# CSRavasio/oflibpytorch

Hardware: AMD Instinct MI355X
Metric: Mpix/s warped+composed (Flow(...) x2 from raw tensors, Flow.apply 't' C=3 + valid area, then Flow.combine_with mode=3 -- the methods combine_flows / apply_flow wrap -- 1080p fp32) (higher is better)
Workload: dtype f32; 1 GPU; B=64/GPU 1080x1920 fp32: Flow(f,'t',mask) x2 (validation), Flow.apply('t', C=3 image, target+flow masks, valid area) + combine_with(mode=3, 't', masks); batch_per_gpu=64, global_batch=64, height=1080, width=1920, parallelism=batch-sharded x1 (no data-path collective), launcher=single process, bytes_per_px=62

## Files before the change

### include/oflib_hip.h

```cpp
#ifndef OFLIB_HIP_H
#define OFLIB_HIP_H

#include <stdint.h>

#ifdef __cplusplus
extern "C" {
#endif

#define OFL_OK 0
#define OFL_E_NULL -1
#define OFL_E_SHAPE -2
#define OFL_E_ARG -3
#define OFL_E_UNSUPPORTED -4

int ofl_version(void);

#define OFL_OPT_WARP_PATH 1
#define OFL_OPT_WARP_SHEAR 3
#define OFL_OPT_SPLAT_PASS_IMAGES 4
#define OFL_OPT_SPLAT_FALLBACK_SLOTS 5
#define OFL_OPT_SPLAT_EXTRA_LDS 7
int ofl_set_option(int32_t key, int32_t value);
const char* ofl_last_kernel_name(void);

// ... 76 lines not shown
                            const uint8_t* chan_mask_a, int64_t chan_mask_a_bs,
                            const uint8_t* chan_mask_b, int64_t chan_mask_b_bs,
                            int32_t with_mask_chan, int32_t occlude,
                            float* dst, float* density, uint8_t* warped, uint8_t* valid, float* mask_chan,
                            int32_t* workspace, int64_t workspace_ints, float* accum_fallback,
                            int32_t n, int32_t c, int32_t h, int32_t w,
                            int32_t round_mode, void* stream);

int ofl_splat_sum_f32(const float* flow, int64_t flow_bs, float flow_sign,
                      const float* data, int64_t data_bs, float data_sign, float* dst,
                      int32_t* workspace, int64_t workspace_ints, float* accum_fallback,
                      int32_t n, int32_t c, int32_t h, int32_t w, void* stream);

#define OFL_FLAG_NONFINITE 1
#define OFL_FLAG_NZ 2
#define OFL_FLAG_NZ_THR 4
#define OFL_FLAG_NZ_MASKED 8
#define OFL_FLAG_NZ_THR_MASKED 16

int ofl_flow_flags_f32(const float* flow, int64_t flow_bs,
                       const uint8_t* mask, int64_t mask_bs, float thr,
                       int32_t* flags, int32_t n, int32_t h, int32_t w, void* stream);

#define OFL_FLAGS_HOST_WORK_EXTRA 33
int ofl_flow_flags_host(const void* flow, int32_t flow_is_f16, int64_t flow_bs,
                        const uint8_t* mask, int64_t mask_bs, float thr,
                        int32_t* work, int32_t* host_words, int32_t serial,
                        int32_t n, int32_t h, int32_t w, void* stream);
int ofl_host_words_alloc(int64_t ints, void** out);
int ofl_host_words_free(void* ptr);

int ofl_flow_from_f16(const void* src_f16, int64_t src_bs,
                      const uint8_t* mask, int64_t mask_bs,
                      float* dst, int32_t* flags,
                      int32_t n, int32_t h, int32_t w, void* stream);
int ofl_splat_tiled_f16(const void* flow_f16, int64_t flow_bs, float flow_sign,
                        const void* data_f16, int64_t data_bs, float data_sign,
                        const uint8_t* weight_mask, int64_t weight_mask_bs,
                        const uint8_t* chan_mask_a, int64_t chan_mask_a_bs,
                        const uint8_t* chan_mask_b, int64_t chan_mask_b_bs,
                        int32_t with_mask_chan, int32_t occlude,
                        void* dst, int32_t dst_is_f16, uint8_t* valid, int32_t* dst_flags,
                        int32_t* workspace, int64_t workspace_ints, float* accum_fallback,
                        int32_t n, int32_t h, int32_t w, void* stream);
int ofl_warp_bwd_h_f32(const float* flow, int64_t flow_bs, float flow_sign,
                       const void* src_f16, int64_t src_bs,
                       const float* src_b, int64_t src_b_bs,
                       const uint8_t* src_mask, int64_t src_mask_bs,
                       const uint8_t* flow_mask, int64_t flow_mask_bs,
                       float* dst, uint8_t* valid,
                       int32_t n, int32_t h, int32_t w, void* stream);

#define OFL_X16_HALF 0
// ... 136 lines not shown
```

### oflibpytorch_amd/_build.py

```python
import os
import shutil
import subprocess

_PKG = os.path.dirname(os.path.abspath(__file__))
_ROOT = os.path.dirname(_PKG)
SOURCES = [os.path.join(_PKG, "csrc", "ofl_kernels.hip"), os.path.join(_PKG, "csrc", "ofl_aux_kernels.hip"), os.path.join(_PKG, "csrc", "ofl_splat_gather.hip"),
           os.path.join(_PKG, "csrc", "ofl_warp_wide.hip"), os.path.join(_PKG, "csrc", "ofl_visualise.hip"), os.path.join(_PKG, "csrc", "ofl_matrix.hip"),
           os.path.join(_PKG, "csrc", "ofl_arrows.hip"), os.path.join(_PKG, "csrc", "ofl_mesh.hip"), os.path.join(_PKG, "csrc", "ofl_warp_half.hip"),
           os.path.join(_PKG, "csrc", "ofl_warp_nhwc.hip"), os.path.join(_PKG, "csrc", "ofl_loaders.hip"), os.path.join(_PKG, "csrc", "ofl_metrics.hip"),
           os.path.join(_PKG, "csrc", "ofl_consistency.hip"),
           os.path.join(_PKG, "csrc", "ofl_png_host.cpp")]
HEADERS = [os.path.join(_ROOT, "include", "oflib_hip.h")]
LIB_PATH = os.path.join(_PKG, "libofl_hip.so")

HIPCC_FLAGS = ["-O3", "--offload-arch=gfx950", "-std=c++17", "-fPIC", "-shared", "-ffp-contract=off",
               "-fno-fast-math", "-fvisibility=hidden"]


def hipcc_path() -> str:
    for cand in (os.environ.get("HIPCC"), shutil.which("hipcc"), "/opt/rocm/bin/hipcc"):
        if cand and os.path.exists(cand):
            return cand
    raise RuntimeError("oflibpytorch_amd: hipcc not found (set HIPCC or install ROCm under /opt/rocm)")


def needs_build() -> bool:
    if not os.path.exists(LIB_PATH):
        return True
    t = os.path.getmtime(LIB_PATH)
    return any(os.path.getmtime(s) > t for s in SOURCES + HEADERS)


def build(force: bool = False, verbose: bool = False) -> str:
    if not force and not needs_build():
# ... 39 lines not shown
```

### oflibpytorch_amd/_native.py

```python
import ctypes
import math
import os
import threading
import time

import numpy as np
import torch

from . import _build

FLAG_NONFINITE, FLAG_NZ, FLAG_NZ_THR, FLAG_NZ_MASKED, FLAG_NZ_THR_MASKED = 1, 2, 4, 8, 16
ABI_VERSION = 36
ROUND_NONE, ROUND_RINT, ROUND_U8 = 0, 1, 2
THRESHOLD = 1e-3

_SYMBOLS = ("ofl_version", "ofl_set_option", "ofl_warp_bwd_f32", "ofl_splat_fwd_f32", "ofl_splat_finalize_f32", "ofl_splat_tiled_workspace_ints", "ofl_splat_tiled_pass_images",
            "ofl_splat_tiled_f32", "ofl_flow_flags_f32", "ofl_warp_bwd_u8", "ofl_flow_from_f16",
            "ofl_warp_bwd_grad_f32", "ofl_splat_grad_f32", "ofl_sample_pts_f32", "ofl_sample_pts_grad_f32",
            "ofl_flow_extents_f32", "ofl_flag_words_or_i32", "ofl_splat_sum_f32", "ofl_warp_bwd_win_f32", "ofl_splat_tiled_win_f32", "ofl_splat_tiled_f16",
            "ofl_warp_bwd_h_f32", "ofl_flow_flags_host", "ofl_host_words_alloc", "ofl_host_words_free", "ofl_flow_from_matrix_f32", "ofl_splat_tiled_fallback_images", "ofl_warp_valid_f32", "ofl_resize_bilinear_f32", "ofl_splat_tile_geometry", "ofl_splat_gather_info", "ofl_last_kernel_name",
            "ofl_visualise_workspace_ints", "ofl_visualise_range_f32", "ofl_visualise_u8",
            "ofl_matrix_workspace_bytes", "ofl_matrix_fit_f64",
            "ofl_arrows_workspace_ints", "ofl_arrows_scale_f32", "ofl_arrows_plan", "ofl_arrows_u8",
            "ofl_mesh_workspace_ints", "ofl_mesh_plan", "ofl_mesh_apply", "ofl_mesh_points",
            "ofl_warp_bwd_x16", "ofl_warp_bwd_grad_x16", "ofl_splat_sum_x16", "ofl_warp_bwd_nhwc",
            "ofl_warp_bwd_grad_nhwc", "ofl_nhwc_to_planes", "ofl_planes_to_nhwc",
            "ofl_png_unfilter", "ofl_png_grey8", "ofl_decode_kitti", "ofl_decode_flo",
            "ofl_flow_error_workspace_bytes", "ofl_flow_error_f64", "ofl_flow_epe_grad_f32",
            "ofl_flow_consistency_workspace_bytes", "ofl_flow_consistency_f32")
_lib = None
_load_lock = threading.RLock()


class NativeUnavailable(RuntimeError):
    """The HIP backend (libofl_hip.so + a visible HIP device) is required and missing."""


def load_library(path: str = None):
    if _lib is not None and path is None:
        return _lib
    with _load_lock:
        return _load_library_locked(path)

# ... 41 lines not shown
    lib.ofl_splat_tiled_pass_images.argtypes = [i32, i32, i32]
    lib.ofl_splat_tiled_fallback_images.argtypes = [i32, i32, i32, i32]
    lib.ofl_splat_tile_geometry.argtypes = [p, p, p]
    lib.ofl_splat_gather_info.argtypes = [i32, i32, i32, i32, i32, p]
    lib.ofl_splat_tiled_f32.argtypes = [p, i64, f32, p, p, i64, p, i64, f32, p, i64, p, i64, p, i64, p, i64, i32, i32, p, p, p, p, p,
                                        p, p, i64, p, i32, i32, i32, i32, i32, p]
    lib.ofl_warp_bwd_grad_f32.argtypes = [p, i64, f32, p, i64, p, f32, p, i64, p, i32, i32, i32, i32, p]
    lib.ofl_splat_grad_f32.argtypes = [p, i64, f32, p, p, i64, p, i64, p, i64, i32, p, p, p, p, p, p, p, i32, i32, i32, i32, p]
    lib.ofl_sample_pts_f32.argtypes = [p, i64, p, i64, p, i32, i32, i32, i32, p]
    lib.ofl_sample_pts_grad_f32.argtypes = [p, i64, p, i64, p, p, p, i32, i32, i32, i32, p]
    lib.ofl_flow_extents_f32.argtypes = [p, i64, p, i64, f32, p, p, i32, i32, i32, p]
    lib.ofl_warp_valid_f32.argtypes = [p, i64, f32, p, i64, f32, p, i32, i32, i32, p]
    lib.ofl_resize_bilinear_f32.argtypes = [p, p, i32, i32, i32, i32, i32, f32, f32, p]
    lib.ofl_flag_words_or_i32.argtypes = [p, i32, p, p]
    lib.ofl_splat_sum_f32.argtypes = [p, i64, f32, p, i64, f32, p, p, i64, p, i32, i32, i32, i32, p]
    lib.ofl_splat_tiled_f16.argtypes = [p, i64, f32, p, i64, f32, p, i64, p, i64, p, i64, i32, i32, p, i32, p, p, p, i64, p, i32, i32, i32, p]
    lib.ofl_warp_bwd_h_f32.argtypes = [p, i64, f32, p, i64, p, i64, p, i64, p, i64, p, p, i32, i32, i32, p]
    lib.ofl_warp_bwd_win_f32.argtypes = [p, i64, f32, i32, i32, i32, i32, p, i64, p, i64, p, i64, p, p, i32, i32, i32, i32, i32, p]
    lib.ofl_splat_tiled_win_f32.argtypes = [p, i64, f32, i32, i32, i32, i32, p, i64, f32, p, i64, p, i64, p, i64, i32, i32, p, p, p, p, p,
                                            p, i64, p, i32, i32, i32, i32, i32, p]
    lib.ofl_flow_flags_host.argtypes = [p, i32, i64, p, i64, f32, p, p, i32, i32, i32, i32, p]
    lib.ofl_host_words_alloc.argtypes = [i64, ctypes.POINTER(ctypes.c_void_p)]
    lib.ofl_host_words_free.argtypes = [p]
    lib.ofl_flow_from_matrix_f32.argtypes = [p, i64, f32, p, i32, i32, i32, p]
    lib.ofl_visualise_workspace_ints.argtypes = [i32]
    lib.ofl_visualise_range_f32.argtypes = [p, i64, i32, p, i64, p, p, p, i32, i32, i32, p]
    lib.ofl_visualise_u8.argtypes = [p, i64, i32, p, i64, i32, i32, p, i32, i32, p, i32, i32, i32, p]
    lib.ofl_matrix_workspace_bytes.argtypes = [i32, i32, i32, i32, i32]
    lib.ofl_matrix_fit_f64.argtypes = [p, i64, i32, i32, p, i64, i32, i32, i32, i32, i32, p, p, p, p]
    lib.ofl_arrows_workspace_ints.argtypes = [i32, i32, i32, i32]
    lib.ofl_arrows_scale_f32.argtypes = [p, i64, i32, i32, p, p, i32, i32, i32, p]
    lib.ofl_arrows_plan.argtypes = [p, i64, i32, i32, i32, p, i32, i32, f32, p, i32, i32, i32, p]
    lib.ofl_arrows_u8.argtypes = [p, i64, i32, p, i64, i32, i32, i32, p, p, i64, i32, p, i32, i32, i32, p]
    lib.ofl_mesh_workspace_ints.argtypes = [i32, i32, i32, i32]
    lib.ofl_mesh_plan.argtypes = [p, i64, f32, p, i64, i32, p, i32, i32, i32, p]
    lib.ofl_mesh_apply.argtypes = [p, i64, f32, p, i64, p, i64, i32, i32, p, p, i64, p, p, p, i32, i32, i32, i32, i32, p]
    lib.ofl_mesh_points.argtypes = [p, i64, f32, p, i64, p, i64, p, p, i64, p, p, i32, i32, i32, i32, p]
    lib.ofl_warp_bwd_x16.argtypes = [p, i64, f32, p, i64, p, i64, p, i64, p, i64, p, i64, f32, f32, p, p, p, p, p,
                                     i32, i32, i32, i32, i32, i32, p]
    lib.ofl_warp_bwd_grad_x16.argtypes = [p, i64, f32, p, i64, p, f32, p, i32, i32, i32, i32, i32, p]
    lib.ofl_splat_sum_x16.argtypes = [p, i64, f32, p, i64, f32, p, p, i64, p, i32, i32, i32, i32, i32, p]
    lib.ofl_warp_bwd_nhwc.argtypes = [p, i64, f32, p, i64, p, i64, p, i64, p, p, i32, i32, i32, i32, i32, p]
    lib.ofl_warp_bwd_grad_nhwc.argtypes = [p, i64, f32, p, i64, p, f32, p, i32, i32, i32, i32, i32, p]
    lib.ofl_nhwc_to_planes.argtypes = [p, p, i32, i32, i32, i32, i32, p]
    lib.ofl_planes_to_nhwc.argtypes = [p, p, i32, i32, i32, i32, i32, p]
    lib.ofl_png_unfilter.argtypes = [p, i64, i32, i32, i32, i32, p, i64]
# ... 119 lines not shown
    lib, dev = load_library(), device(vecs, mask)
    n, _, h, w = vecs.shape
    if vecs.dtype == torch.float16 and vecs.device.type == 'cuda':
        with _on(dev):
            v, vbs = _planes(vecs.detach(), dev, torch.float16, n, "flow")
            if vbs != 0 or n == 1:
                m, mbs = (None, 0) if mask is None else _planes(mask, dev, torch.bool, n, "mask")
                flags = torch.zeros(n, dtype=torch.int32, device=dev)
                rc = lib.ofl_flow_from_f16(_ptr(v), vbs, _ptr(m), mbs, None, _ptr(flags), n, h, w, _stream(dev))
                if rc != -4:
                    _check(rc, "ofl_flow_from_f16")
                    return flags
        vecs = vecs.float()
    with _on(dev):
        v, vbs = _planes(vecs.detach(), dev, torch.float32, n, "flow")
        m, mbs = (None, 0) if mask is None else _planes(mask, dev, torch.bool, n, "mask")
        flags = torch.zeros(n, dtype=torch.int32, device=dev)
        _check(lib.ofl_flow_flags_f32(_ptr(v), vbs, _ptr(m), mbs, THRESHOLD, _ptr(flags), n, h, w, _stream(dev)),
               "ofl_flow_flags_f32")
    return flags


_HOST_WORDS = 1 << 12
_WORK_EXTRA = 33
_MAX_SLOTS = 8
_host_slots = {}
_host_slots_lock = threading.Lock()
_SPIN_SLACK_SECONDS = 150e-6
_YIELD_SECONDS = 20e-3
HOST_POLL_SECONDS = 20.0


def _new_host_slot(lib, dev):
    addr = ctypes.c_void_p()
    with torch.cuda.device(dev):
        _check(lib.ofl_host_words_alloc(2 * _HOST_WORDS, ctypes.byref(addr)), "ofl_host_words_alloc")
        work = torch.zeros(_HOST_WORDS + _WORK_EXTRA, dtype=torch.int32, device=dev)
    view = np.ctypeslib.as_array((ctypes.c_int32 * (2 * _HOST_WORDS)).from_address(addr.value))
    return [threading.Lock(), work, addr, view, 0, False]


def _acquire_host_slot(lib, dev):
    while True:
        slots = _host_slots.get(dev.index)
        if slots is not None:
            for slot in tuple(slots):
                if slot[0].acquire(False):
                    if slot[5]:
                        slot[0].release()
                        continue
                    return slot
        with _host_slots_lock:
            slots = _host_slots.setdefault(dev.index, [])
            if len(slots) < _MAX_SLOTS:
                slot = _new_host_slot(lib, dev)
                slot[0].acquire()
                slots.append(slot)
                return slot
            busy = slots[0]
        busy[0].acquire()
        if not busy[5]:
            return busy
# ... 13 lines not shown
        return None
    n, _, h, w = vecs.shape
    if n > _HOST_WORDS:
        return None
    lib, dev = load_library(), vecs.device
    half = vecs.dtype == torch.float16
    switch = torch.cuda.current_device() != dev.index
    ctx = torch.cuda.device(dev) if switch else None
    if ctx is not None:
        ctx.__enter__()
    try:
        if vecs.is_contiguous() and (mask is None or (mask.dtype == torch.bool and mask.device == dev and mask.shape[0] == n
                                                      and mask.is_contiguous())):
            v, vbs, m, mbs = vecs, 2 * h * w, mask, h * w
        else:
            v, vbs = _planes(vecs.detach(), dev, vecs.dtype, n, "flow")
            if half and vbs == 0 and n != 1:
                return None
            m, mbs = (None, 0) if mask is None else _planes(mask, dev, torch.bool, n, "mask")
        slot = _acquire_host_slot(lib, dev)
        stream = torch._C._cuda_getCurrentRawStream(dev.index)
        try:
            serial = slot[4] = (slot[4] % 0x7ffffff0) + 1
            view = slot[3]
            rc = lib.ofl_flow_flags_host(v.data_ptr(), 1 if half else 0, vbs, 0 if m is None else m.data_ptr(), mbs, THRESHOLD,
                                         slot[1].data_ptr(), slot[2], serial, n, h, w, stream)
            if rc == -4:
                return None
            _check(rc, "ofl_flow_flags_host")
            try:
                tags = view[0:2 * n:2]
                t0 = time.perf_counter()
                spin_until = t0 + 2.0 * (n * h * w * (5 if half else 9)) / 4e12 + _SPIN_SLACK_SECONDS
                looks = 0
                while not (view[2 * n - 2] == serial and (n == 1 or bool((tags == serial).all()))):
                    looks += 1
                    if looks & 0x3f == 0:
                        now = time.perf_counter()
                        if now > spin_until:
                            time.sleep(0 if now - t0 < _YIELD_SECONDS else 5e-5)
                            if now - t0 > HOST_POLL_SECONDS:
                                torch.cuda.synchronize(dev)
                                if bool((tags == serial).all()):
                                    break
                                raise RuntimeError("oflibpytorch_amd: the flag reduction did not report back")
                return view[1:2 * n:2].tolist()
            except BaseException:
                try:
                    torch.cuda.synchronize(dev)
                finally:
                    _drop_host_slot(dev, slot)
                raise
        finally:
            slot[0].release()
    finally:
        if ctx is not None:
            ctx.__exit__(None, None, None)


def flow_from_half(vecs16: torch.Tensor, mask: torch.Tensor = None):
    lib, dev = load_library(), device(vecs16, mask)
    n, _, h, w = vecs16.shape
    if _wants_grad(vecs16):
        dst = vecs16.to(dev).float()
        return dst, flow_flags(dst, mask)
    with _on(dev):
        v, vbs = _planes(vecs16, dev, torch.float16, n, "flow")
        if vbs != 0 or n == 1:
            m, mbs = (None, 0) if mask is None else _planes(mask, dev, torch.bool, n, "mask")
# ... 1034 lines not shown
```

### oflibpytorch_amd/csrc/ofl_kernels.hip

```cpp
#include <hip/hip_runtime.h>
#include <stdint.h>
#include <type_traits>

#include "oflib_hip.h"

#pragma clang fp contract(off)

int ofl_wide_launch_column(const void* params, int nc, void* stream);
int ofl_wide_launch_rows(const void* params, int nc, int tiles, void* stream);
int ofl_wide_launch_rows_h(const void* params, void* stream);
int ofl_wide_launch_rows_grad(const void* params, int nc, int tiles, void* stream);
int ofl_wide_launch_rows_u8(const void* params, int nc, int dst_is_u8, void* stream);
int ofl_wide_launch_chan(const void* params, int rows, void* stream);
int ofl_warp_path_option(void);
int ofl_warp_shear_option(void);
int ofl_splat_launch_gather_diet(const void* params, int nc, int mch, int elem, unsigned grid, void* stream, int extra_lds);

extern const void* g_ofl_last_kernel;
#define OFL_KLAUNCH(K, ...) do { g_ofl_last_kernel = (const void*)(K); hipLaunchKernelGGL(K, __VA_ARGS__); } while (0)

namespace {

constexpr float kValidThr = 0.99999f;
constexpr float kZeroThr = 1e-3f;
// ... 3043 lines not shown
            a0 = b0; b0 = min(a0 + span, ub);
        }
    }
    if (NC == 2 && s.dst_flags) {
        dflags = wave_or_flags(dflags);
        block_flag_or(&s.dst_flags[n], dflags);
    }
    if (!REDO) break;
#if OFL_SP2_UNITTIME
    if (tid == 0) {
        const uint64_t t1 = wall_clock64();
        p.redo_list[2 * ri] = tile | ((uint32_t)((unit_t0 >> 3) & 0xffffu) << 16);
        p.redo_list[2 * ri + 1] = (uint32_t)ua | ((uint32_t)ub << 8) | ((uint32_t)min((t1 - unit_t0) >> 2, (uint64_t)0xffffu) << 16);
    }
#endif
    if (tid == 0) next_unit = (int)gridDim.x + atomicAdd(&p.redo_cnt[1], 1);
    __syncthreads();
    ri = __builtin_amdgcn_readfirstlane(next_unit);
    } while (ri < redo_n);
#undef s
#undef p
}

constexpr int kFlagShards = 32;
struct FlagsHost { int32_t* counters; unsigned long long* host; int32_t serial, total_blocks, n; };

__device__ __forceinline__ void flags_publish(int32_t* __restrict__ flags, const FlagsHost& fh) {
    __shared__ int last;
    asm volatile("s_waitcnt vmcnt(0)" ::: "memory");
    __syncthreads();
    if (threadIdx.x == 0) {
        const int id = (int)(blockIdx.y * gridDim.x + blockIdx.x), shard = id % kFlagShards;
        const int in_shard = (fh.total_blocks - shard + kFlagShards - 1) / kFlagShards;
        const int shards = fh.total_blocks < kFlagShards ? fh.total_blocks : kFlagShards;
        int l = 0;
        if (__hip_atomic_fetch_add(fh.counters + shard, 1, __ATOMIC_RELAXED, __HIP_MEMORY_SCOPE_AGENT) == in_shard - 1)
            l = __hip_atomic_fetch_add(fh.counters + kFlagShards, 1, __ATOMIC_RELAXED, __HIP_MEMORY_SCOPE_AGENT) == shards - 1;
        last = l;
    }
    __syncthreads();
    if (!last) return;
    if (threadIdx.x <= kFlagShards) {
        const int old = __hip_atomic_exchange(fh.counters + threadIdx.x, 0, __ATOMIC_RELAXED, __HIP_MEMORY_SCOPE_AGENT);
        asm volatile("" :: "v"(old));
    }
    asm volatile("s_waitcnt vmcnt(0)" ::: "memory");
    __syncthreads();
    for (int i = threadIdx.x; i < fh.n; i += blockDim.x) {
        const uint32_t v = (uint32_t)__hip_atomic_exchange(&flags[i], 0, __ATOMIC_RELAXED, __HIP_MEMORY_SCOPE_AGENT);
        __hip_atomic_store(&fh.host[i], ((unsigned long long)v << 32) | (uint32_t)fh.serial, __ATOMIC_RELAXED, __HIP_MEMORY_SCOPE_SYSTEM);
    }
}

template <bool VEC, bool NT = false, bool HOST = false>
__global__ __launch_bounds__(256) void flow_flags_kernel(const float* __restrict__ flow, int64_t flow_bs,
                                                         const uint8_t* __restrict__ mask, int64_t mask_bs,
                                                         int32_t* __restrict__ flags, int64_t hw, const FlagsHost fh) {
    const int n = blockIdx.y;
    const float* fu = flow + n * flow_bs;
    const uint8_t* mk = mask ? mask + n * mask_bs : nullptr;
    int f = 0;
    const int64_t stride = (int64_t)gridDim.x * blockDim.x;
    if (VEC) {
        const int64_t hw4 = hw >> 2;
        constexpr int R = 4;
        bool skip_mask = false;
        for (int64_t i0 = (int64_t)blockIdx.x * blockDim.x + threadIdx.x; i0 < hw4; i0 += R * stride) {
            f4 a[R], b[R]; uint32_t m4[R];
#pragma unroll
            for (int r = 0; r < R; ++r) {
                const int64_t i = i0 + r * stride;
                if (i < hw4) {
                    if (NT) { a[r] = ld4nt(fu + 4 * i); b[r] = ld4nt(fu + hw + 4 * i); }
                    else { a[r] = reinterpret_cast<const f4*>(fu)[i]; b[r] = reinterpret_cast<const f4*>(fu + hw)[i]; }
                    m4[r] = (mk && !skip_mask) ? reinterpret_cast<const uint32_t*>(mk)[i] : 0x01010101u;
                }
            }
#pragma unroll
            for (int r = 0; r < R; ++r) {
                if (i0 + r * stride < hw4) {
#pragma unroll
                    for (int k = 0; k < 4; ++k) f |= flag_bits(a[r][k], b[r][k], ((m4[r] >> (8 * k)) & 0xffu) != 0u);
                }
            }
            if (mk && !skip_mask) skip_mask = __any((f & OFL_FLAG_NZ_THR_MASKED) != 0) != 0;
        }
    } else {
        for (int64_t i = (int64_t)blockIdx.x * blockDim.x + threadIdx.x; i < hw; i += stride)
            f |= flag_bits(fu[i], fu[hw + i], mk ? (mk[i] != 0) : true);
    }
    f = wave_or_flags(f);
    block_flag_or(&flags[n], f);
    if (HOST) flags_publish(flags, fh);
}

typedef _Float16 h4 __attribute__((ext_vector_type(4)));
template <bool HOST = false>
__global__ __launch_bounds__(256) void flow_f16_kernel(const _Float16* __restrict__ src, int64_t src_bs,
                                                       const uint8_t* __restrict__ mask, int64_t mask_bs,
                                                       float* __restrict__ dst, int32_t* __restrict__ flags, int64_t hw, const FlagsHost fh) {
    const int n = blockIdx.y;
    const _Float16* su = src + n * src_bs;
    float* du = dst + (int64_t)n * 2 * hw;
    const uint8_t* mk = mask ? mask + n * mask_bs : nullptr;
    int f = 0;
    const int64_t stride = (int64_t)gridDim.x * blockDim.x, hw4 = hw >> 2;
    for (int64_t i0 = (int64_t)blockIdx.x * blockDim.x + threadIdx.x; i0 < hw4; i0 += 4 * stride) {
        h4 a[4], b[4]; uint32_t m4[4];
#pragma unroll
        for (int r = 0; r < 4; ++r) {
            const int64_t i = i0 + r * stride;
            if (i < hw4) {
                a[r] = reinterpret_cast<const h4*>(su)[i]; b[r] = reinterpret_cast<const h4*>(su + hw)[i];
                m4[r] = mk ? reinterpret_cast<const uint32_t*>(mk)[i] : 0x01010101u;
            }
        }
#pragma unroll
        for (int r = 0; r < 4; ++r) {
            const int64_t i = i0 + r * stride;
            if (i < hw4) {
                const f4 u = {(float)a[r][0], (float)a[r][1], (float)a[r][2], (float)a[r][3]};
                const f4 v = {(float)b[r][0], (float)b[r][1], (float)b[r][2], (float)b[r][3]};
                if (dst) { reinterpret_cast<f4*>(du)[i] = u; reinterpret_cast<f4*>(du + hw)[i] = v; }
#pragma unroll
                for (int k = 0; k < 4; ++k) f |= flag_bits(u[k], v[k], ((m4[r] >> (8 * k)) & 0xffu) != 0u);
            }
        }
    }
    f = wave_or_flags(f);
    block_flag_or(&flags[n], f);
    if (HOST) flags_publish(flags, fh);
}

inline int check_dims(int32_t n, int32_t c, int32_t h, int32_t w, bool splat = true) {
    if (n < 1 || c < 1 || h < 1 || w < 1) return OFL_E_SHAPE;
    if (splat && (int64_t)h * w >= (1ll << 24)) return OFL_E_SHAPE;
    if ((int64_t)h * w >= (1ll << 31)) return OFL_E_SHAPE;
    return OFL_OK;
}

inline void tile_grid(int32_t n, int32_t h, int32_t w, int32_t& tiles_x, int32_t& tiles_y, int64_t& total,
                      int64_t& per_xcd, unsigned& grid) {
    tiles_x = (w + kTileW - 1) / kTileW;
    tiles_y = (h + kTileH - 1) / kTileH;
    total = (int64_t)tiles_x * tiles_y * n;
    per_xcd = (total + kXcds - 1) / kXcds;
    grid = (unsigned)(per_xcd * kXcds);
}

inline void magic_u32(uint32_t d, uint32_t& m, uint32_t& s) {
    uint32_t l = 0;
    while ((1ull << l) < d) ++l;
    m = (uint32_t)(((1ull << 32) * ((1ull << l) - d)) / d + 1);
    s = ((l ? 1u : 0u) << 16) | (l ? l - 1 : 0);
// ... 473 lines not shown
    return (int)hipGetLastError();
}

template <int NC, typename TD>
int launch_warp_lds_u8(WarpParams& q, hipStream_t st) {
    const unsigned g = warp_geometry(q, kLdsTWQ * 4, 2 * kLdsTH);
    OFL_WITH_BOOL(q.valid != nullptr, V, OFL_KLAUNCH((warp_bwd_lds_kernel<NC, V, false, false, false, uint8_t, TD>), dim3(g), dim3(kLdsNT), kLdsBytes, st, q));
    return (int)hipGetLastError();
}

inline bool aligned_to(const void* ptr, size_t a) { return (reinterpret_cast<uintptr_t>(ptr) % a) == 0; }

#ifndef OFL_FLAGS_BLOCKS
#define OFL_FLAGS_BLOCKS 512
#endif
void launch_flow_flags(const float* flow, int64_t flow_bs, const uint8_t* mask, int64_t mask_bs, int32_t* flags, int32_t n,
                       int64_t hw, hipStream_t st, const FlagsHost* fhp = nullptr) {
    const bool vec = (hw % 4) == 0 && aligned_to(flow, 16) && (flow_bs % 4) == 0 && (!mask || (aligned_to(mask, 4) && (mask_bs % 4) == 0));
    FlagsHost fh = {};
    if (fhp) fh = *fhp;
    if (vec) {
        int64_t bx = (hw / 4 + 1023) / 1024;
        int64_t cap = (n <= 8 ? OFL_FLAGS_BLOCKS / 2 : OFL_FLAGS_BLOCKS) / n;
        cap = cap < 16 ? 16 : (cap > 256 ? 256 : cap);
        if (bx > cap) bx = cap;
        fh.total_blocks = (int32_t)(bx * n);
        const bool nt = 9 * hw * n >= ((int64_t)256 << 20);
        if (fhp) {
            if (nt) OFL_KLAUNCH((flow_flags_kernel<true, true, true>), dim3((unsigned)bx, (unsigned)n), dim3(256), 0, st, flow, flow_bs, mask, mask_bs, flags, hw, fh);
            else OFL_KLAUNCH((flow_flags_kernel<true, false, true>), dim3((unsigned)bx, (unsigned)n), dim3(256), 0, st, flow, flow_bs, mask, mask_bs, flags, hw, fh);
        } else {
            if (nt) OFL_KLAUNCH((flow_flags_kernel<true, true>), dim3((unsigned)bx, (unsigned)n), dim3(256), 0, st, flow, flow_bs, mask, mask_bs, flags, hw, fh);
            else OFL_KLAUNCH((flow_flags_kernel<true, false>), dim3((unsigned)bx, (unsigned)n), dim3(256), 0, st, flow, flow_bs, mask, mask_bs, flags, hw, fh);
        }
    } else {
        int64_t bx = (hw + 255) / 256;
        if (bx > 512) bx = 512;
        fh.total_blocks = (int32_t)(bx * n);
        if (fhp) OFL_KLAUNCH((flow_flags_kernel<false, false, true>), dim3((unsigned)bx, (unsigned)n), dim3(256), 0, st, flow, flow_bs, mask, mask_bs, flags, hw, fh);
        else OFL_KLAUNCH((flow_flags_kernel<false>), dim3((unsigned)bx, (unsigned)n), dim3(256), 0, st, flow, flow_bs, mask, mask_bs, flags, hw, fh);
    }
}

template <int CT>
int launch_warp(const WarpParams& p, unsigned grid, hipStream_t st) {
    const bool valid = p.valid != nullptr, add = p.addend != nullptr, flags = p.flow_flags != nullptr;
    OFL_WITH_BOOL(valid, V, OFL_WITH_BOOL(add, A, OFL_WITH_BOOL(flags, F, OFL_KLAUNCH((warp_bwd_kernel<CT, V, A, F>), dim3(grid), dim3(256), 0, st, p))));
    return (int)hipGetLastError();
}


inline unsigned fallback_resident_blocks(const void* kernel, int which) {
    static int cache[64][11];
    int dev = 0;
    if (hipGetDevice(&dev) != hipSuccess || dev < 0 || dev >= 64) dev = 0;
    int v = cache[dev][which];
    if (v == 0) {
        int per_cu = 0, cus = 0;
        if (hipOccupancyMaxActiveBlocksPerMultiprocessor(&per_cu, kernel, 256, 0) != hipSuccess) per_cu = 1;
        if (hipDeviceGetAttribute(&cus, hipDeviceAttributeMultiprocessorCount, dev) != hipSuccess || cus < 1) cus = 1;
        if (per_cu > 1) per_cu -= 1;
// ... 592 lines not shown
    if (n > 65535) return OFL_E_SHAPE;
    const int64_t hw = (int64_t)h * w;
    if ((hw % 4) != 0 || !aligned_to(src_f16, 8) || (src_bs % 4) != 0 || (dst && !aligned_to(dst, 16)) ||
        (mask && (!aligned_to(mask, 4) || (mask_bs % 4) != 0)))
        return OFL_E_UNSUPPORTED;
    int64_t bx = (hw / 4 + 1023) / 1024, cap = 512 / n;
    cap = cap < 16 ? 16 : (cap > 256 ? 256 : cap);
    if (bx > cap) bx = cap;
    OFL_KLAUNCH(flow_f16_kernel<false>, dim3((unsigned)bx, (unsigned)n), dim3(256), 0, (hipStream_t)stream,
                       static_cast<const _Float16*>(src_f16), src_bs, mask, mask_bs, dst, flags, hw, FlagsHost{});
    return (int)hipGetLastError();
}

__attribute__((visibility("default"))) int ofl_flow_flags_host(const void* flow, int32_t flow_is_f16, int64_t flow_bs,
                                                               const uint8_t* mask, int64_t mask_bs, float thr,
                                                               int32_t* work, int32_t* host_words, int32_t serial,
                                                               int32_t n, int32_t h, int32_t w, void* stream) {
    if (!flow || !work || !host_words) return OFL_E_NULL;
    int rc = check_dims(n, 2, h, w, false);
    if (rc) return rc;
    if (n > 65535) return OFL_E_SHAPE;
    if (thr != kZeroThr) return OFL_E_ARG;
    const int64_t hw = (int64_t)h * w;
    if ((reinterpret_cast<uintptr_t>(host_words) & 7) != 0) return OFL_E_ARG;
    FlagsHost fh = {};
    fh.counters = work + n; fh.host = reinterpret_cast<unsigned long long*>(host_words); fh.serial = serial; fh.n = n;
    hipStream_t st = (hipStream_t)stream;
    if (!flow_is_f16) {
        launch_flow_flags(static_cast<const float*>(flow), flow_bs, mask, mask_bs, work, n, hw, st, &fh);
        return (int)hipGetLastError();
    }
    if ((hw % 4) != 0 || !aligned_to(flow, 8) || (flow_bs % 4) != 0 || (mask && (!aligned_to(mask, 4) || (mask_bs % 4) != 0)))
        return OFL_E_UNSUPPORTED;
    int64_t bx = (hw / 4 + 1023) / 1024, cap = 512 / n;
    cap = cap < 16 ? 16 : (cap > 256 ? 256 : cap);
    if (bx > cap) bx = cap;
    fh.total_blocks = (int32_t)(bx * n);
    OFL_KLAUNCH(flow_f16_kernel<true>, dim3((unsigned)bx, (unsigned)n), dim3(256), 0, st,
                       static_cast<const _Float16*>(flow), flow_bs, mask, mask_bs, (float*)nullptr, work, hw, fh);
    return (int)hipGetLastError();
}

__attribute__((visibility("default"))) int ofl_host_words_alloc(int64_t ints, void** out) {
    if (!out || ints < 1) return OFL_E_ARG;
    void* ptr = nullptr;
    hipError_t e = hipHostMalloc(&ptr, (size_t)ints * sizeof(int32_t), hipHostMallocCoherent | hipHostMallocMapped);
    if (e != hipSuccess) return (int)e;
    for (int64_t i = 0; i < ints; ++i) static_cast<volatile int32_t*>(ptr)[i] = 0;
    *out = ptr;
    return OFL_OK;
}
__attribute__((visibility("default"))) int ofl_host_words_free(void* ptr) { return ptr ? (int)hipHostFree(ptr) : OFL_OK; }

}
#endif
```

### oflibpytorch_amd/distributed.py

```python
import atexit
import threading
import time

import numpy as np
import torch
import torch.distributed as dist

_group = None
_enabled = False
_force_collectives = False
_exchange = None
USE_HOST_EXCHANGE = True
EXCHANGE_TIMEOUT_SECONDS = None


class _HostExchange(object):
    RING = 4

    def __init__(self, group):
        from multiprocessing import shared_memory
        self.rank, self.world = dist.get_rank(group), dist.get_world_size(group)
        self.seq = 0
        self.lock = threading.Lock()
        self.group = group
        size = self.world * self.RING * 8
        name = [None]
        self.shm = None
        if self.rank == 0:
            try:
                self.shm = shared_memory.SharedMemory(create=True, size=size)
                np.ndarray((self.world * self.RING,), dtype=np.int64, buffer=self.shm.buf)[:] = 0
                name[0] = self.shm.name
            except Exception:
                self.shm = None
        dist.broadcast_object_list(name, src=dist.get_global_rank(group, 0) if group is not None else 0, group=group)
        ok = 1 if name[0] is not None else 0
        if self.rank != 0 and ok:
            try:
                self.shm = shared_memory.SharedMemory(name=name[0])
                try:
                    from multiprocessing import resource_tracker
                    resource_tracker.unregister(self.shm._name, "shared_memory")
                except Exception:
                    pass
            except Exception:
                ok = 0
        flag = torch.tensor([ok], dtype=torch.int32, device=_collective_device(group))
        dist.all_reduce(flag, op=dist.ReduceOp.MIN, group=group)
        self.usable = bool(int(flag.cpu()[0]))
        self.slots = None if self.shm is None else np.ndarray((self.world, self.RING), dtype=np.int64, buffer=self.shm.buf)

    def or_reduce(self, bits: int) -> int:
        with self.lock:
            return self._or_reduce_locked(bits)

    def _or_reduce_locked(self, bits: int) -> int:
        self.seq += 1
        k, e = self.seq, self.seq % self.RING
        self.slots[self.rank, e] = (k << 8) | (bits & 0xff)
        total, t0, looks, timeout = bits & 0xff, None, 0, None
        for r in range(self.world):
            if r == self.rank:
                continue
            while True:
                v = int(self.slots[r, e])
                if (v >> 8) == k:
                    total |= v & 0xff
                    break
                looks += 1
                if looks & 0x3ff == 0 or t0 is not None:
                    now = time.perf_counter()
                    t0 = now if t0 is None else t0
                    if timeout is None:
                        timeout = _exchange_timeout(self.group)
                    if now - t0 > timeout:
                        raise RuntimeError("oflibpytorch_amd.distributed: rank %d did not post flag exchange %d within %.0f s (ranks "
                                           "must make the same sequence of calls; EXCHANGE_TIMEOUT_SECONDS overrides the process "
                                           "group's timeout)" % (r, k, timeout))
                    if now - t0 > 1e-3:
                        time.sleep(5e-5 if now - t0 < 1.0 else 1e-3)
        return total

    def close(self):
        shm, self.shm, self.slots = self.shm, None, None
        if shm is not None:
            try:
                shm.close()
                if self.rank == 0:
                    shm.unlink()
            except Exception:
                pass


def _exchange_timeout(group) -> float:
    if EXCHANGE_TIMEOUT_SECONDS is not None:
        return float(EXCHANGE_TIMEOUT_SECONDS)
    try:
        pg = group if group is not None else dist.group.WORLD
        return float(pg._get_backend(_collective_device(group)).options._timeout.total_seconds())
    except Exception:
        pass
    try:
        return float(dist.distributed_c10d._get_default_timeout(dist.get_backend(group)).total_seconds())
    except Exception:
        return 1800.0


# ... 118 lines not shown
```

### oflibpytorch_amd/flow_class.py

```python
import math
import warnings
import weakref
from typing import Tuple, Union

import numpy as np
import torch
import torch.nn.functional as F

from . import _consistency, _native, distributed
from .utils import (get_valid_vecs, get_valid_ref, get_valid_mask, get_valid_device, get_valid_padding,
                    get_valid_shape, get_pure_pytorch, move_axis, from_matrix, from_transforms, resize_flow,
                    apply_flow, _flags_to_host, _host_flags, _griddata_unavailable, track_pts, get_half_flow_outputs,
                    interpolate_bilinear, _mesh_mode)

FlowAlias = 'Flow'
_VALID_THR = 0.99999
_COMBINE_FUSED = True


class _NeverEqual(object):
    __slots__ = ()

    def __eq__(self, other):
        return False
# ... 150 lines not shown
        obj._device = obj._vecs.device
        obj.ref = ref
        if mask is not None:
            m = get_valid_mask(mask, desired_shape=obj.shape, error_string="Error setting flow mask: ")
            obj._mask = m.to(obj._vecs.device)
        obj.device = device
        return obj

    def _key(self) -> tuple:
        return (_ver(self._fv, self._private), None if self._mask is None else (id(self._mask), _ver(self._mask, self._private)), _reval_epoch)

    def _flags_known(self) -> bool:
        key = self._key()
        return self._flag_cache is not None and self._flag_cache[0] == key

    def _flags(self) -> list:
        key = self._key()
        if self._flag_cache is None or self._flag_cache[0] != key:
            dev_flags = None
            if self._pending_flags is not None and self._pending_flags[0] == key:
                dev_flags = self._pending_flags[1]
            self._pending_flags = None
            sharded = distributed.is_enabled()
            if dev_flags is None and (not sharded or distributed.host_exchange_active()):
                words = _host_flags(self._fv, self._mask)
                self._flag_cache = (key, words)
                if sharded:
                    local = 0
                    for f in words:
                        local |= f
                    self._flag_cache = (key, words, (True, distributed.reduce_flags(local, self._fv.device)))
                return self._flag_cache[1]
            if dev_flags is None:
                dev_flags = _native.flow_flags(self._fv, self._mask)
            if sharded and distributed.host_exchange_active():
                words = _flags_to_host(dev_flags)
                local = 0
                for f in words:
                    local |= f
                self._flag_cache = (key, words, (True, distributed.reduce_flags(local, self._fv.device)))
            elif sharded:
                words, glob = distributed.split_global_or(_flags_to_host(distributed.with_global_or(dev_flags)))
                self._flag_cache = (key, words, (True, glob))
            else:
                self._flag_cache = (key, _flags_to_host(dev_flags))
        return self._flag_cache[1]

    def _set_pending_flags(self, dev_flags):
        if dev_flags is not None:
            key = self._key()
            self._pending_flags = (key, dev_flags)

    def _batch_flags(self) -> int:
        flags = self._flags()
        if len(self._flag_cache) < 3 or self._flag_cache[2][0] != distributed.is_enabled():
# ... 989 lines not shown
```

Measured before the change: 67500 Mpix/s.

## Pack per-image flag counts into 64-bit atomics and wait for host flags natively

```diff
diff --git a/include/oflib_hip.h b/include/oflib_hip.h
--- a/include/oflib_hip.h
+++ b/include/oflib_hip.h
@@ -122,13 +122,16 @@
                        const uint8_t* mask, int64_t mask_bs, float thr,
                        int32_t* flags, int32_t n, int32_t h, int32_t w, void* stream);
 
-#define OFL_FLAGS_HOST_WORK_EXTRA 33
 int ofl_flow_flags_host(const void* flow, int32_t flow_is_f16, int64_t flow_bs,
                         const uint8_t* mask, int64_t mask_bs, float thr,
                         int32_t* work, int32_t* host_words, int32_t serial,
                         int32_t n, int32_t h, int32_t w, void* stream);
 int ofl_host_words_alloc(int64_t ints, void** out);
 int ofl_host_words_free(void* ptr);
+int ofl_flags_wait(const void* host_words, int32_t n, int32_t serial, int64_t spin_ns, int64_t budget_ns, int64_t sleep_ns,
+                   int32_t* words);
+int ofl_flags_exchange(void* segment, int32_t world, int32_t ring, int32_t rank, int64_t seq, int32_t bits, int64_t spin_ns,
+                       int64_t budget_ns, int64_t sleep_ns, int32_t* result);
 
 int ofl_flow_from_f16(const void* src_f16, int64_t src_bs,
                       const uint8_t* mask, int64_t mask_bs,
diff --git a/oflibpytorch_amd/_build.py b/oflibpytorch_amd/_build.py
--- a/oflibpytorch_amd/_build.py
+++ b/oflibpytorch_amd/_build.py
@@ -9,7 +9,7 @@
            os.path.join(_PKG, "csrc", "ofl_arrows.hip"), os.path.join(_PKG, "csrc", "ofl_mesh.hip"), os.path.join(_PKG, "csrc", "ofl_warp_half.hip"),
            os.path.join(_PKG, "csrc", "ofl_warp_nhwc.hip"), os.path.join(_PKG, "csrc", "ofl_loaders.hip"), os.path.join(_PKG, "csrc", "ofl_metrics.hip"),
            os.path.join(_PKG, "csrc", "ofl_consistency.hip"),
-           os.path.join(_PKG, "csrc", "ofl_png_host.cpp")]
+           os.path.join(_PKG, "csrc", "ofl_png_host.cpp"), os.path.join(_PKG, "csrc", "ofl_flags_wait.cpp")]
 HEADERS = [os.path.join(_ROOT, "include", "oflib_hip.h")]
 LIB_PATH = os.path.join(_PKG, "libofl_hip.so")
 
diff --git a/oflibpytorch_amd/_native.py b/oflibpytorch_amd/_native.py
--- a/oflibpytorch_amd/_native.py
+++ b/oflibpytorch_amd/_native.py
@@ -18,7 +18,7 @@
             "ofl_splat_tiled_f32", "ofl_flow_flags_f32", "ofl_warp_bwd_u8", "ofl_flow_from_f16",
             "ofl_warp_bwd_grad_f32", "ofl_splat_grad_f32", "ofl_sample_pts_f32", "ofl_sample_pts_grad_f32",
             "ofl_flow_extents_f32", "ofl_flag_words_or_i32", "ofl_splat_sum_f32", "ofl_warp_bwd_win_f32", "ofl_splat_tiled_win_f32", "ofl_splat_tiled_f16",
-            "ofl_warp_bwd_h_f32", "ofl_flow_flags_host", "ofl_host_words_alloc", "ofl_host_words_free", "ofl_flow_from_matrix_f32", "ofl_splat_tiled_fallback_images", "ofl_warp_valid_f32", "ofl_resize_bilinear_f32", "ofl_splat_tile_geometry", "ofl_splat_gather_info", "ofl_last_kernel_name",
+            "ofl_warp_bwd_h_f32", "ofl_flow_flags_host", "ofl_host_words_alloc", "ofl_host_words_free", "ofl_flags_wait", "ofl_flags_exchange", "ofl_flow_from_matrix_f32", "ofl_splat_tiled_fallback_images", "ofl_warp_valid_f32", "ofl_resize_bilinear_f32", "ofl_splat_tile_geometry", "ofl_splat_gather_info", "ofl_last_kernel_name",
             "ofl_visualise_workspace_ints", "ofl_visualise_range_f32", "ofl_visualise_u8",
             "ofl_matrix_workspace_bytes", "ofl_matrix_fit_f64",
             "ofl_arrows_workspace_ints", "ofl_arrows_scale_f32", "ofl_arrows_plan", "ofl_arrows_u8",
@@ -106,6 +106,8 @@
     lib.ofl_flow_flags_host.argtypes = [p, i32, i64, p, i64, f32, p, p, i32, i32, i32, i32, p]
     lib.ofl_host_words_alloc.argtypes = [i64, ctypes.POINTER(ctypes.c_void_p)]
     lib.ofl_host_words_free.argtypes = [p]
+    lib.ofl_flags_wait.argtypes = [p, i32, i32, i64, i64, i64, p]
+    lib.ofl_flags_exchange.argtypes = [p, i32, i32, i32, i64, i32, i64, i64, i64, p]
     lib.ofl_flow_from_matrix_f32.argtypes = [p, i64, f32, p, i32, i32, i32, p]
     lib.ofl_visualise_workspace_ints.argtypes = [i32]
     lib.ofl_visualise_range_f32.argtypes = [p, i64, i32, p, i64, p, p, p, i32, i32, i32, p]
@@ -271,12 +273,13 @@
 
 
 _HOST_WORDS = 1 << 12
-_WORK_EXTRA = 33
 _MAX_SLOTS = 8
 _host_slots = {}
 _host_slots_lock = threading.Lock()
 _SPIN_SLACK_SECONDS = 150e-6
 _YIELD_SECONDS = 20e-3
+_WAIT_SLEEP_NS = 50000
+_WAIT_SLICE_NS = 2000000
 HOST_POLL_SECONDS = 20.0
 
 
@@ -284,9 +287,9 @@
     addr = ctypes.c_void_p()
     with torch.cuda.device(dev):
         _check(lib.ofl_host_words_alloc(2 * _HOST_WORDS, ctypes.byref(addr)), "ofl_host_words_alloc")
-        work = torch.zeros(_HOST_WORDS + _WORK_EXTRA, dtype=torch.int32, device=dev)
+        work = torch.zeros(_HOST_WORDS, dtype=torch.int64, device=dev)
     view = np.ctypeslib.as_array((ctypes.c_int32 * (2 * _HOST_WORDS)).from_address(addr.value))
-    return [threading.Lock(), work, addr, view, 0, False]
+    return [threading.Lock(), work, addr, view, 0, False, (ctypes.c_int32 * _HOST_WORDS)()]
 
 
 def _acquire_host_slot(lib, dev):
@@ -346,29 +349,28 @@
         stream = torch._C._cuda_getCurrentRawStream(dev.index)
         try:
             serial = slot[4] = (slot[4] % 0x7ffffff0) + 1
-            view = slot[3]
+            words = slot[6]
             rc = lib.ofl_flow_flags_host(v.data_ptr(), 1 if half else 0, vbs, 0 if m is None else m.data_ptr(), mbs, THRESHOLD,
                                          slot[1].data_ptr(), slot[2], serial, n, h, w, stream)
             if rc == -4:
                 return None
             _check(rc, "ofl_flow_flags_host")
             try:
-                tags = view[0:2 * n:2]
                 t0 = time.perf_counter()
-                spin_until = t0 + 2.0 * (n * h * w * (5 if half else 9)) / 4e12 + _SPIN_SLACK_SECONDS
-                looks = 0
-                while not (view[2 * n - 2] == serial and (n == 1 or bool((tags == serial).all()))):
-                    looks += 1
-                    if looks & 0x3f == 0:
-                        now = time.perf_counter()
-                        if now > spin_until:
-                            time.sleep(0 if now - t0 < _YIELD_SECONDS else 5e-5)
-                            if now - t0 > HOST_POLL_SECONDS:
-                                torch.cuda.synchronize(dev)
-                                if bool((tags == serial).all()):
-                                    break
-                                raise RuntimeError("oflibpytorch_amd: the flag reduction did not report back")
-                return view[1:2 * n:2].tolist()
+                spin_ns = int((2.0 * (n * h * w * (5 if half else 9)) / 4e12 + _SPIN_SLACK_SECONDS) * 1e9)
+                wait, pairs = lib.ofl_flags_wait, slot[2]
+                rc = wait(pairs, n, serial, spin_ns, spin_ns + _WAIT_SLICE_NS, 0, words)
+                while rc == 0:
+                    waited = time.perf_counter() - t0
+                    if waited > HOST_POLL_SECONDS:
+                        torch.cuda.synchronize(dev)
+                        if wait(pairs, n, serial, 0, 0, 0, words) == 1:
+                            break
+                        raise RuntimeError("oflibpytorch_amd: the flag reduction did not report back")
+                    rc = wait(pairs, n, serial, 0, _WAIT_SLICE_NS, 0 if waited < _YIELD_SECONDS else _WAIT_SLEEP_NS, words)
+                if rc < 0:
+                    _check(rc, "ofl_flags_wait")
+                return words[:n]
             except BaseException:
                 try:
                     torch.cuda.synchronize(dev)
diff --git a/oflibpytorch_amd/csrc/ofl_flags_wait.cpp b/oflibpytorch_amd/csrc/ofl_flags_wait.cpp
--- /dev/null
+++ b/oflibpytorch_amd/csrc/ofl_flags_wait.cpp
@@ -0,0 +1,110 @@
+#include <stdint.h>
+#include <sched.h>
+#include <time.h>
+
+#include "oflib_hip.h"
+
+#define OFL_EXPORT extern "C" __attribute__((visibility("default")))
+
+namespace {
+
+constexpr int32_t kMaxWords = 1 << 12;
+constexpr int32_t kMaxWorld = 1 << 10;
+constexpr int64_t kMaxSeq = (int64_t)1 << 54;
+constexpr int kLooksPerClock = 64;
+
+inline void cpu_relax() {
+#if defined(__x86_64__) || defined(__i386__)
+    __builtin_ia32_pause();
+#elif defined(__aarch64__)
+    __asm__ __volatile__("yield");
+#endif
+}
+
+inline int64_t now_ns() {
+    timespec ts;
+    clock_gettime(CLOCK_MONOTONIC, &ts);
+    return (int64_t)ts.tv_sec * 1000000000 + ts.tv_nsec;
+}
+
+inline void rest(int64_t ns) {
+    if (ns <= 0) {
+        sched_yield();
+        return;
+    }
+    timespec ts;
+    ts.tv_sec = (time_t)(ns / 1000000000);
+    ts.tv_nsec = (long)(ns % 1000000000);
+    nanosleep(&ts, nullptr);
+}
+
+template <typename Look>
+inline int paced(Look look, int64_t spin_ns, int64_t budget_ns, int64_t sleep_ns) {
+    if (look()) return 1;
+    if (budget_ns <= 0) return 0;
+    const int64_t t0 = now_ns();
+    const int64_t spin_end = t0 + (spin_ns < budget_ns ? spin_ns : budget_ns), end = t0 + budget_ns;
+    int64_t now = t0;
+    while (now < spin_end) {
+        for (int i = 0; i < kLooksPerClock; ++i) {
+            cpu_relax();
+            if (look()) return 1;
+        }
+        now = now_ns();
+    }
+    while (now < end) {
+        rest(sleep_ns);
+        if (look()) return 1;
+        now = now_ns();
+    }
+    return 0;
+}
+
+}
+
+OFL_EXPORT int ofl_flags_wait(const void* host_words, int32_t n, int32_t serial, int64_t spin_ns, int64_t budget_ns, int64_t sleep_ns,
+                              int32_t* words) {
+    if (!host_words || !words) return OFL_E_NULL;
+    if (n < 1 || n > kMaxWords) return OFL_E_SHAPE;
+    if (((uintptr_t)host_words & 7) != 0 || spin_ns < 0 || budget_ns < 0 || sleep_ns < 0) return OFL_E_ARG;
+    const uint64_t* pairs = (const uint64_t*)host_words;
+    const uint32_t tag = (uint32_t)serial;
+    int32_t seen = 0;
+    auto look = [&]() -> bool {
+        while (seen < n) {
+            const uint64_t v = __atomic_load_n(pairs + seen, __ATOMIC_ACQUIRE);
+            if ((uint32_t)v != tag) return false;
+            words[seen++] = (int32_t)(uint32_t)(v >> 32);
+        }
+        return true;
+    };
+    return paced(look, spin_ns, budget_ns, sleep_ns);
+}
+
+OFL_EXPORT int ofl_flags_exchange(void* segment, int32_t world, int32_t ring, int32_t rank, int64_t seq, int32_t bits, int64_t spin_ns,
+                                  int64_t budget_ns, int64_t sleep_ns, int32_t* result) {
+    if (!segment || !result) return OFL_E_NULL;
+    if (world < 1 || world > kMaxWorld || ring < 2 || ring > 1024) return OFL_E_SHAPE;
+    if (((uintptr_t)segment & 7) != 0 || rank < 0 || rank >= world || seq < 1 || seq >= kMaxSeq || bits < 0 || bits > 0xff ||
+        spin_ns < 0 || budget_ns < 0 || sleep_ns < 0)
+        return OFL_E_ARG;
+    int64_t* slots = (int64_t*)segment;
+    const int64_t e = seq % ring;
+    __atomic_store_n(slots + (int64_t)rank * ring + e, (seq << 8) | bits, __ATOMIC_RELEASE);
+    int32_t total = bits, r = 0;
+    auto look = [&]() -> bool {
+        while (r < world) {
+            if (r != rank) {
+                const int64_t v = __atomic_load_n(slots + (int64_t)r * ring + e, __ATOMIC_ACQUIRE);
+                if ((v >> 8) != seq) return false;
+                total |= (int32_t)(v & 0xff);
+            }
+            ++r;
+        }
+        return true;
+    };
+    const int done = paced(look, spin_ns, budget_ns, sleep_ns);
+    result[0] = total;
+    result[1] = done ? -1 : r;
+    return done;
+}
diff --git a/oflibpytorch_amd/csrc/ofl_kernels.hip b/oflibpytorch_amd/csrc/ofl_kernels.hip
--- a/oflibpytorch_amd/csrc/ofl_kernels.hip
+++ b/oflibpytorch_amd/csrc/ofl_kernels.hip
@@ -3089,34 +3089,32 @@
 #undef p
 }
 
-constexpr int kFlagShards = 32;
-struct FlagsHost { int32_t* counters; unsigned long long* host; int32_t serial, total_blocks, n; };
-
-__device__ __forceinline__ void flags_publish(int32_t* __restrict__ flags, const FlagsHost& fh) {
-    __shared__ int last;
-    asm volatile("s_waitcnt vmcnt(0)" ::: "memory");
+constexpr int kArriveBits = 14, kBitCountBits = 10, kFlagBits = 5;
+constexpr int kFlagsVecBlockCap = 256, kFlagsScalarBlockCap = 512;
+static_assert(kArriveBits + kFlagBits * kBitCountBits <= 64, "an image's work word is one 64-bit atomic");
+static_assert(kFlagsVecBlockCap < (1 << kBitCountBits) && kFlagsScalarBlockCap < (1 << kBitCountBits) && kFlagsScalarBlockCap < (1 << kArriveBits),
+              "a counter of the work word must hold every block of an image");
+struct FlagsHost { unsigned long long* work; unsigned long long* host; int32_t serial; };
+
+__device__ __forceinline__ void flags_publish(int image, int f, const FlagsHost& fh) {
+    __shared__ int bflags;
+    if (threadIdx.x == 0) bflags = 0;
     __syncthreads();
-    if (threadIdx.x == 0) {
-        const int id = (int)(blockIdx.y * gridDim.x + blockIdx.x), shard = id % kFlagShards;
-        const int in_shard = (fh.total_blocks - shard + kFlagShards - 1) / kFlagShards;
-        const int shards = fh.total_blocks < kFlagShards ? fh.total_blocks : kFlagShards;
-        int l = 0;
-        if (__hip_atomic_fetch_add(fh.counters + shard, 1, __ATOMIC_RELAXED, __HIP_MEMORY_SCOPE_AGENT) == in_shard - 1)
-            l = __hip_atomic_fetch_add(fh.counters + kFlagShards, 1, __ATOMIC_RELAXED, __HIP_MEMORY_SCOPE_AGENT) == shards - 1;
-        last = l;
-    }
+    if ((threadIdx.x & 63) == 0 && f != 0) atomicOr(&bflags, f);
     __syncthreads();
-    if (!last) return;
-    if (threadIdx.x <= kFlagShards) {
-        const int old = __hip_atomic_exchange(fh.counters + threadIdx.x, 0, __ATOMIC_RELAXED, __HIP_MEMORY_SCOPE_AGENT);
-        asm volatile("" :: "v"(old));
-    }
-    asm volatile("s_waitcnt vmcnt(0)" ::: "memory");
-    __syncthreads();
-    for (int i = threadIdx.x; i < fh.n; i += blockDim.x) {
-        const uint32_t v = (uint32_t)__hip_atomic_exchange(&flags[i], 0, __ATOMIC_RELAXED, __HIP_MEMORY_SCOPE_AGENT);
-        __hip_atomic_store(&fh.host[i], ((unsigned long long)v << 32) | (uint32_t)fh.serial, __ATOMIC_RELAXED, __HIP_MEMORY_SCOPE_SYSTEM);
-    }
+    if (threadIdx.x != 0) return;
+    const int bf = bflags;
+    unsigned long long add = 1ull;
+#pragma unroll
+    for (int b = 0; b < kFlagBits; ++b) add |= (unsigned long long)((bf >> b) & 1) << (kArriveBits + kBitCountBits * b);
+    const unsigned long long before = __hip_atomic_fetch_add(fh.work + image, add, __ATOMIC_RELAXED, __HIP_MEMORY_SCOPE_AGENT);
+    if ((before & ((1ull << kArriveBits) - 1)) != (unsigned long long)(gridDim.x - 1)) return;
+    const unsigned long long sums = __hip_atomic_exchange(fh.work + image, 0ull, __ATOMIC_RELAXED, __HIP_MEMORY_SCOPE_AGENT);
+    uint32_t v = 0;
+#pragma unroll
+    for (int b = 0; b < kFlagBits; ++b)
+        if (((sums >> (kArriveBits + kBitCountBits * b)) & ((1ull << kBitCountBits) - 1)) != 0ull) v |= 1u << b;
+    __hip_atomic_store(&fh.host[image], ((unsigned long long)v << 32) | (uint32_t)fh.serial, __ATOMIC_RELAXED, __HIP_MEMORY_SCOPE_SYSTEM);
 }
 
 template <bool VEC, bool NT = false, bool HOST = false>
@@ -3157,8 +3155,8 @@
             f |= flag_bits(fu[i], fu[hw + i], mk ? (mk[i] != 0) : true);
     }
     f = wave_or_flags(f);
-    block_flag_or(&flags[n], f);
-    if (HOST) flags_publish(flags, fh);
+    if (HOST) flags_publish(n, f, fh);
+    else block_flag_or(&flags[n], f);
 }
 
 typedef _Float16 h4 __attribute__((ext_vector_type(4)));
@@ -3195,8 +3193,8 @@
         }
     }
     f = wave_or_flags(f);
-    block_flag_or(&flags[n], f);
-    if (HOST) flags_publish(flags, fh);
+    if (HOST) flags_publish(n, f, fh);
+    else block_flag_or(&flags[n], f);
 }
 
 inline int check_dims(int32_t n, int32_t c, int32_t h, int32_t w, bool splat = true) {
@@ -3716,9 +3714,8 @@
     if (vec) {
         int64_t bx = (hw / 4 + 1023) / 1024;
         int64_t cap = (n <= 8 ? OFL_FLAGS_BLOCKS / 2 : OFL_FLAGS_BLOCKS) / n;
-        cap = cap < 16 ? 16 : (cap > 256 ? 256 : cap);
+        cap = cap < 16 ? 16 : (cap > kFlagsVecBlockCap ? kFlagsVecBlockCap : cap);
         if (bx > cap) bx = cap;
-        fh.total_blocks = (int32_t)(bx * n);
         const bool nt = 9 * hw * n >= ((int64_t)256 << 20);
         if (fhp) {
             if (nt) OFL_KLAUNCH((flow_flags_kernel<true, true, true>), dim3((unsigned)bx, (unsigned)n), dim3(256), 0, st, flow, flow_bs, mask, mask_bs, flags, hw, fh);
@@ -3729,8 +3726,7 @@
         }
     } else {
         int64_t bx = (hw + 255) / 256;
-        if (bx > 512) bx = 512;
-        fh.total_blocks = (int32_t)(bx * n);
+        if (bx > kFlagsScalarBlockCap) bx = kFlagsScalarBlockCap;
         if (fhp) OFL_KLAUNCH((flow_flags_kernel<false, false, true>), dim3((unsigned)bx, (unsigned)n), dim3(256), 0, st, flow, flow_bs, mask, mask_bs, flags, hw, fh);
         else OFL_KLAUNCH((flow_flags_kernel<false>), dim3((unsigned)bx, (unsigned)n), dim3(256), 0, st, flow, flow_bs, mask, mask_bs, flags, hw, fh);
     }
@@ -4369,9 +4365,9 @@
     if (n > 65535) return OFL_E_SHAPE;
     if (thr != kZeroThr) return OFL_E_ARG;
     const int64_t hw = (int64_t)h * w;
-    if ((reinterpret_cast<uintptr_t>(host_words) & 7) != 0) return OFL_E_ARG;
+    if ((reinterpret_cast<uintptr_t>(host_words) & 7) != 0 || (reinterpret_cast<uintptr_t>(work) & 7) != 0) return OFL_E_ARG;
     FlagsHost fh = {};
-    fh.counters = work + n; fh.host = reinterpret_cast<unsigned long long*>(host_words); fh.serial = serial; fh.n = n;
+    fh.work = reinterpret_cast<unsigned long long*>(work); fh.host = reinterpret_cast<unsigned long long*>(host_words); fh.serial = serial;
     hipStream_t st = (hipStream_t)stream;
     if (!flow_is_f16) {
         launch_flow_flags(static_cast<const float*>(flow), flow_bs, mask, mask_bs, work, n, hw, st, &fh);
@@ -4380,9 +4376,8 @@
     if ((hw % 4) != 0 || !aligned_to(flow, 8) || (flow_bs % 4) != 0 || (mask && (!aligned_to(mask, 4) || (mask_bs % 4) != 0)))
         return OFL_E_UNSUPPORTED;
     int64_t bx = (hw / 4 + 1023) / 1024, cap = 512 / n;
-    cap = cap < 16 ? 16 : (cap > 256 ? 256 : cap);
+    cap = cap < 16 ? 16 : (cap > kFlagsVecBlockCap ? kFlagsVecBlockCap : cap);
     if (bx > cap) bx = cap;
-    fh.total_blocks = (int32_t)(bx * n);
     OFL_KLAUNCH(flow_f16_kernel<true>, dim3((unsigned)bx, (unsigned)n), dim3(256), 0, st,
                        static_cast<const _Float16*>(flow), flow_bs, mask, mask_bs, (float*)nullptr, work, hw, fh);
     return (int)hipGetLastError();
diff --git a/oflibpytorch_amd/distributed.py b/oflibpytorch_amd/distributed.py
--- a/oflibpytorch_amd/distributed.py
+++ b/oflibpytorch_amd/distributed.py
@@ -1,4 +1,5 @@
 import atexit
+import ctypes
 import threading
 import time
 
@@ -11,6 +12,8 @@
 _force_collectives = False
 _exchange = None
 USE_HOST_EXCHANGE = True
+_EXCHANGE_SPIN_NS = 1000000
+_EXCHANGE_SLICE_SECONDS = 5e-3
 EXCHANGE_TIMEOUT_SECONDS = None
 
 
@@ -20,6 +23,12 @@
     def __init__(self, group):
         from multiprocessing import shared_memory
         self.rank, self.world = dist.get_rank(group), dist.get_world_size(group)
+        try:
+            from . import _native
+            self._fn = _native.load_library().ofl_flags_exchange
+        except Exception:
+            self._fn = None
+        self._result = (ctypes.c_int32 * 2)()
         self.seq = 0
         self.lock = threading.Lock()
         self.group = group
@@ -34,7 +43,7 @@
             except Exception:
                 self.shm = None
         dist.broadcast_object_list(name, src=dist.get_global_rank(group, 0) if group is not None else 0, group=group)
-        ok = 1 if name[0] is not None else 0
+        ok = 1 if name[0] is not None and self._fn is not None else 0
         if self.rank != 0 and ok:
             try:
                 self.shm = shared_memory.SharedMemory(name=name[0])
@@ -49,6 +58,7 @@
         dist.all_reduce(flag, op=dist.ReduceOp.MIN, group=group)
         self.usable = bool(int(flag.cpu()[0]))
         self.slots = None if self.shm is None else np.ndarray((self.world, self.RING), dtype=np.int64, buffer=self.shm.buf)
+        self._base = None if self.slots is None else ctypes.c_void_p(self.slots.ctypes.data)
 
     def or_reduce(self, bits: int) -> int:
         with self.lock:
@@ -56,33 +66,24 @@
 
     def _or_reduce_locked(self, bits: int) -> int:
         self.seq += 1
-        k, e = self.seq, self.seq % self.RING
-        self.slots[self.rank, e] = (k << 8) | (bits & 0xff)
-        total, t0, looks, timeout = bits & 0xff, None, 0, None
-        for r in range(self.world):
-            if r == self.rank:
-                continue
-            while True:
-                v = int(self.slots[r, e])
-                if (v >> 8) == k:
-                    total |= v & 0xff
-                    break
-                looks += 1
-                if looks & 0x3ff == 0 or t0 is not None:
-                    now = time.perf_counter()
-                    t0 = now if t0 is None else t0
-                    if timeout is None:
-                        timeout = _exchange_timeout(self.group)
-                    if now - t0 > timeout:
-                        raise RuntimeError("oflibpytorch_amd.distributed: rank %d did not post flag exchange %d within %.0f s (ranks "
-                                           "must make the same sequence of calls; EXCHANGE_TIMEOUT_SECONDS overrides the process "
-                                           "group's timeout)" % (r, k, timeout))
-                    if now - t0 > 1e-3:
-                        time.sleep(5e-5 if now - t0 < 1.0 else 1e-3)
-        return total
+        k, bits, res, fn = self.seq, bits & 0xff, self._result, self._fn
+        rc = fn(self._base, self.world, self.RING, self.rank, k, bits, _EXCHANGE_SPIN_NS, _EXCHANGE_SPIN_NS, 0, res)
+        if rc == 0:
+            t0, timeout = time.perf_counter(), _exchange_timeout(self.group)
+            while rc == 0:
+                waited = time.perf_counter() - t0
+                if waited > timeout:
+                    raise RuntimeError("oflibpytorch_amd.distributed: rank %d did not post flag exchange %d within %.0f s (ranks "
+                                       "must make the same sequence of calls; EXCHANGE_TIMEOUT_SECONDS overrides the process "
+                                       "group's timeout)" % (res[1], k, timeout))
+                slice_ns = int(min(_EXCHANGE_SLICE_SECONDS, timeout - waited) * 1e9) + 1
+                rc = fn(self._base, self.world, self.RING, self.rank, k, bits, 0, slice_ns, 50000 if waited < 1.0 else 1000000, res)
+        if rc < 0:
+            raise RuntimeError("oflibpytorch_amd.distributed: ofl_flags_exchange failed with code %d" % rc)
+        return res[0]
 
     def close(self):
-        shm, self.shm, self.slots = self.shm, None, None
+        shm, self.shm, self.slots, self._base = self.shm, None, None, None
         if shm is not None:
             try:
                 shm.close()
diff --git a/oflibpytorch_amd/flow_class.py b/oflibpytorch_amd/flow_class.py
--- a/oflibpytorch_amd/flow_class.py
+++ b/oflibpytorch_amd/flow_class.py
@@ -196,15 +196,17 @@
                 dev_flags = self._pending_flags[1]
             self._pending_flags = None
             sharded = distributed.is_enabled()
-            if dev_flags is None and (not sharded or distributed.host_exchange_active()):
+            exchange = distributed._exchange if sharded else None
+            if dev_flags is None and (not sharded or exchange is not None):
                 words = _host_flags(self._fv, self._mask)
-                self._flag_cache = (key, words)
-                if sharded:
+                if exchange is None:
+                    self._flag_cache = (key, words)
+                else:
                     local = 0
                     for f in words:
                         local |= f
-                    self._flag_cache = (key, words, (True, distributed.reduce_flags(local, self._fv.device)))
-                return self._flag_cache[1]
+                    self._flag_cache = (key, words, (True, exchange.or_reduce(local)))
+                return words
             if dev_flags is None:
                 dev_flags = _native.flow_flags(self._fv, self._mask)
             if sharded and distributed.host_exchange_active():
```

After: 67300 Mpix/s. No clear change (-0.3%).
